# WhatAShot/Electrocardio-Panorama

Measured on AMD Instinct MI355X. Metric: ECG-samples/sec (train step), higher is better.
Workload: dtype f32 (conv products: fp32 operands split into fp16 hi+lo = 22-23 bits, block-scaled, 3 fp16 matrix products each, fp32 accumulate; fp32-class, not IEEE fp32)

## Files before the change

### electrocardio_panorama_amd/_lib.py

```python
import ctypes as C
import os

import torch

_HERE = os.path.dirname(os.path.abspath(__file__))
LIB_PATH = os.path.join(_HERE, "csrc", "libnefnet_hip.so")

NEF_OK = 0
_ERR = {-1: "NEF_E_SHAPE", -2: "NEF_E_NULL", -3: "NEF_E_WORKSPACE", -4: "NEF_E_UNSUPPORTED"}

p = C.c_void_p
i32 = C.c_int
i64 = C.c_int64
f32 = C.c_float
sz = C.c_size_t


class ConvArgs(C.Structure):
    _fields_ = [
        ("x", p), ("wp", p), ("y", p), ("bias", p), ("in_scale", p), ("res", p), ("gate", p), ("mask", p),
        ("x_bs", i64), ("x_gs", i64), ("y_bs", i64), ("y_gs", i64), ("sc_bs", i64), ("sc_gs", i64),
        ("res_bs", i64), ("res_gs", i64), ("gate_bs", i64), ("gate_gs", i64),
        ("B", i32), ("T", i32), ("G", i32), ("Cin_g", i32), ("Cout_g", i32), ("K", i32),
        ("relu", i32), ("gate_scale", f32), ("drop_scale", f32), ("drop_p", f32), ("rng_seed", C.c_uint64),
# ... 46 lines not shown
    "nef_convt2_bwd_weight_ws_bytes": (sz, [i32, i32, i32]),
    "nef_convt2_bwd_weight": (i32, [p, p, p, p, p, sz, i32, i32, i32, i32, i32, p]),
    "nef_theta_mlp_fwd": (i32, [p, p, p, p, i32, i32, p]),
    "nef_theta_mlp_bwd": (i32, [p, p, p, p, i32, i32, p]),
    "nef_theta_encode": (i32, [p, p, i32, p]),
    "nef_chscale_fwd": (i32, [p, p, i64, p, i32, i32, i32, p]),
    "nef_chscale_bwd": (i32, [p, p, p, i64, p, p, i32, i32, i32, i32, p]),
    "nef_gate": (i32, [p, p, p, f32, i64, p]),
    "nef_add": (i32, [p, p, p, i64, p]),
    "nef_roi_align_fwd": (i32, [p, p, p, i32, i32, i32, i32, i32, p]),
    "nef_roi_align_bwd": (i32, [p, p, p, i32, i32, i32, i32, i32, p]),
    "nef_window_crop": (i32, [p, i64, i64, p, i32, i32, i32, i32, i32, i32, p]),
    "nef_window_scatter": (i32, [p, p, i64, i64, i32, i32, i32, i32, i32, i32, p]),
    "nef_roi_unpool_fwd": (i32, [p, p, p, p, i32, i32, i32, p]),
    "nef_roi_unpool_bwd": (i32, [p, p, p, i32, i32, i32, p]),
    "nef_roi_segment_table": (i32, [p, p, p, i32, p]),
    "nef_lead_mean": (i32, [p, p, p, i32, i32, i32, p]),
    "nef_mix_fwd": (i32, [p, p, p, p, p, i32, i32, i32, i32, i32, p, p]),
    "nef_mix_bwd": (i32, [p, p, p, p, p, p, p, p, i32, i32, i32, i32, i32, p, i32, p]),
    "nef_mix_fwd_shared": (i32, [p, p, p, p, p, i32, i32, i32, i32, i32, p, p]),
    "nef_lead_mean_mix_shared": (i32, [p, p, p, p, p, i32, i32, i32, i32, i32, p, p]),
    "nef_mix_bwd_shared_up": (i32, [p, p, p, p, p, p, p, p, i32, i32, i32, i32, i32, p, i32, p]),
    "nef_mix_bwd_shared": (i32, [p, p, p, p, p, p, p, p, i32, i32, i32, i32, i32, p, i32, p]),
    "nef_pass_combine_fwd": (i32, [p, p, p, i32, i32, i32, p]),
    "nef_pass_combine_bwd": (i32, [p, p, i32, i32, i32, p]),
    "nef_pass_combine_stats_ws_bytes": (sz, [i32, i32]),
    "nef_pass_combine_fwd_stats": (i32, [p, p, p, p, p, p, p, p, p, p, p, p, sz, i32, i32, i32, f32, f32, p, p]),
    "nef_mix_bwd_up": (i32, [p, p, p, p, p, p, p, p, i32, i32, i32, i32, i32, p, i32, p]),
    "nef_upsample2_fwd": (i32, [p, p, i64, i32, p]),
    "nef_upsample2_bwd": (i32, [p, p, i64, i32, p]),
    "nef_bn_ws_bytes": (sz, [i32, i32]),
    "nef_bn_train_stats": (i32, [p, p, p, p, p, p, p, p, p, p, sz, i32, i32, i32, i32, f32, f32, p, p]),
    "nef_conv_stats_slots": (i32, [i32, i32]),
    "nef_bn_stats_from_slots": (i32, [p, i32, p, p, p, p, p, p, p, p, p, sz, i32, i32, i32, i32, f32, f32, p, p]),
    "nef_bn_eval_affine": (i32, [p, p, p, p, p, p, i32, f32, p]),
    "nef_fold_bn": (i32, [p, p, p, p, p, p, i32, i32, p]),
    "nef_affine_relu_fwd": (i32, [p, p, p, p, i32, i32, i32, i32, p]),
    "nef_bn_bwd_ws_bytes": (sz, [i32, i32, i32]),
    "nef_bn_relu_bwd": (i32, [p, p, p, p, p, p, p, p, p, p, p, p, sz, i32, i32, i32, i32, p, i32, p]),
    "nef_bn_relu_bwd_phase_major": (i32, [p, p, p, p, p, p, p, p, p, p, p, p, sz, i32, i32, i32, i32, p, i32, p]),
    "nef_bn_relu_bwd_up": (i32, [p, p, p, p, p, p, p, p, p, p, p, sz, i32, i32, i32, i32, p, i32, p]),
    "nef_bn_relu_bwd_combine3": (i32, [p, p, p, p, p, p, p, p, p, p, p, sz, i32, i32, i32, p, i32, p]),
    "nef_bn_relu_bwd_combine3_phase_major": (i32, [p, p, p, p, p, p, p, p, p, p, p, sz, i32, i32, i32, p, i32, p]),
    "nef_bn_bwd_outconv_ws_bytes": (sz, [i32, i32, i32, i32]),
    "nef_bn_relu_bwd_outconv": (i32, [p, p, p, p, p, p, p, p, p, p, p, p, p, sz, i32, i32, i32, i32, p]),
    "nef_outconv_fwd": (i32, [p, p, p, p, i32, i32, i32, p]),
# ... 65 lines not shown
```

### electrocardio_panorama_amd/csrc/roi.hip

```cpp
#include "nef_common.h"

namespace {

constexpr int NSEG = NEF_N_SEG;
constexpr int BINS = NEF_ROI_BINS;
constexpr int SEGW = 2 * NEF_ROI_BINS;

__device__ __forceinline__ int64_t latent_index(int64_t roi) {
    return (int64_t)((float)roi * 0.25f);
}

__device__ __forceinline__ float grid_x(const int64_t* __restrict__ roi_b, int j, int s, int T) {
    const float sc = (float)(2.0 / (double)T);
    const float r0 = ((float)roi_b[2 * j] * 0.25f) * sc + (-1.0f);
    const float r1 = ((float)roi_b[2 * j + 1] * 0.25f) * sc + (-1.0f);
    const float step = (r1 - r0) / (float)(BINS - 1);
    return s < BINS / 2 ? r0 + step * (float)s : r1 - step * (float)(BINS - 1 - s);
}

__device__ __forceinline__ float col_weight(float gx) {
    const float ix = ((gx + 1.f) * 1.f - 1.f) * 0.5f;
    const float x0 = floorf(ix);
    const float we = ix - x0;
    const float ww = 1.f - we;
// ... 71 lines not shown
        if (len < 0) { ok = false; len = 0; }
        if (run + len > T) { ok = false; len = T - run; }
        st.start[j] = (int)a;
        st.len[j] = (int)len;
        st.off[j] = run;
        st.scale[j] = len > 0 ? (float)SEGW / (float)(int)len : 0.f;
        run += (int)len;
    }
    if (run != T) ok = false;
    return ok;
}

__device__ __forceinline__ void lerp_src(int i, float scale, int& i0, int& i1, float& l0, float& l1) {
    float src = scale * ((float)i + 0.5f) - 0.5f;
    if (src < 0.f) src = 0.f;
    i0 = (int)src;
    if (i0 > SEGW - 1) i0 = SEGW - 1;
    i1 = i0 + (i0 < SEGW - 1 ? 1 : 0);
    l1 = src - (float)i0;
    if (l1 < 0.f) l1 = 0.f;
    if (l1 > 1.f) l1 = 1.f;
    l0 = 1.f - l1;
}

__global__ void roi_unpool_fwd_kernel(const float* __restrict__ zseg, const int64_t* __restrict__ rois,
                                      float* __restrict__ out, int32_t* __restrict__ status, int B, int C, int T) {
    const int64_t rows = (int64_t)B * C;
    const int wave = __builtin_amdgcn_readfirstlane((int)(threadIdx.x >> 6)), lane = threadIdx.x & 63;
    const int64_t per_wave = (rows + (int64_t)gridDim.x * 4 - 1) / ((int64_t)gridDim.x * 4);
    const int64_t row_lo = ((int64_t)blockIdx.x * 4 + wave) * per_wave;
    const int64_t row_hi = row_lo + per_wave < rows ? row_lo + per_wave : rows;
    int b_cur = -1;
    SegTable st;
    for (int64_t row = row_lo; row < row_hi; ++row) {
        const int b = (int)(row / C);
        if (b != b_cur) {
            b_cur = b;
            const bool ok = load_segments(rois + (int64_t)b * NSEG * 2, T, st);
            if (!ok && status && lane == 0) status[0] = 1;
        }
        const float* zr = zseg + row * NSEG * SEGW;
        float* orow = out + row * T;
        float r[4];
#pragma unroll
        for (int q = 0; q < 4; ++q) r[q] = (q * 64 + lane < NSEG * SEGW) ? zr[q * 64 + lane] : 0.f;
        int covered = 0;
#pragma unroll
        for (int j = 0; j < NSEG; ++j) {
            const int len = st.len[j], off = st.off[j];
            const float sc = st.scale[j];
            const float reg = r[j >> 1];
            const int base = (j & 1) * SEGW;
            for (int ib = 0; ib < len; ib += 64) {
                const int i = ib + lane;
                int i0, i1;
                float l0, l1;
                lerp_src(i, sc, i0, i1, l0, l1);
                const float v0 = __shfl(reg, base + i0), v1 = __shfl(reg, base + i1);
                if (i < len) orow[off + i] = l0 * v0 + l1 * v1;
            }
            covered = off + len;
        }
        for (int t = covered + lane; t < T; t += 64) orow[t] = 0.f;
    }
}

__device__ __forceinline__ int unpool_left_tap(int i, float scale) {
    float src = scale * ((float)i + 0.5f) - 0.5f;
    if (src < 0.f) src = 0.f;
    return (int)src;
}

__device__ __forceinline__ int unpool_first_reaching(int s, int len, float scale, float inv_scale) {
    if (s <= 0) return 0;
    int i = (int)ceilf(((float)s + 0.5f) * inv_scale - 0.5f);
    if (i < 0) i = 0;
    if (i > len) i = len;
    if (i > 0 && unpool_left_tap(i - 1, scale) >= s) --i;
    else if (i < len && unpool_left_tap(i, scale) < s) ++i;
    if ((i > 0 && unpool_left_tap(i - 1, scale) >= s) || (i < len && unpool_left_tap(i, scale) < s)) {
#pragma nounroll
        while (i > 0 && unpool_left_tap(i - 1, scale) >= s) --i;
// ... 54 lines not shown
                const int b1 = s + 1 < SEGW ? nb : len;
                const int a0 = s > 0 ? pb : b0;
                const float* gp = gr + off;
                float fi = (float)a0 + 0.5f;
                const float sm1 = (float)(s - 1);
                for (int i = a0; i < b0; ++i, fi += 1.f) {
                    float src = sc * fi - 0.5f;
                    src = src < 0.f ? 0.f : src;
                    acc += (src - sm1) * gp[i];
                }
                const float c0 = s == SEGW - 1 ? 1.f : (float)(s + 1), k = s == SEGW - 1 ? 0.f : 1.f;
                for (int i = b0; i < b1; ++i, fi += 1.f) {
                    float src = sc * fi - 0.5f;
                    src = src < 0.f ? 0.f : src;
                    acc += (c0 - k * src) * gp[i];
                }
            }
            gz[j * SEGW + s] = acc;
        }
        if constexpr (STAGED) __builtin_amdgcn_wave_barrier();
    }
}

__global__ void roi_segment_table_kernel(const int64_t* __restrict__ rois, int64_t* __restrict__ seg_start,
                                         int64_t* __restrict__ seg_len, int n) {
    const int i = blockIdx.x * blockDim.x + threadIdx.x;
    if (i >= n) return;
    const int64_t a = latent_index(rois[2 * i]);
    const int64_t e = latent_index(rois[2 * i + 1]);
    seg_start[i] = a;
    seg_len[i] = e - a;
}

}

#define NEF_ST ((hipStream_t)stream)

extern "C" {

static bool window_covers_taps(int T, int zT, int t_off) {
    const int r0 = (T - 1) / 2, r1 = (r0 + 1 < T) ? r0 + 1 : r0;
    return zT > 0 && t_off >= 0 && t_off <= r0 && r1 < t_off + zT && t_off + zT <= T;
}

int nef_roi_align_fwd(const float* z, const int64_t* rois, float* out, int B, int C, int T, int zT, int t_off,
                      nef_stream_t stream) {
// ... 20 lines not shown
                       nef_stream_t stream) {
    NEF_ENTER();
    NEF_REQUIRE(zseg && rois && out, NEF_E_NULL);
    NEF_REQUIRE(B > 0 && C > 0 && T > 0, NEF_E_SHAPE);
    hipLaunchKernelGGL(roi_unpool_fwd_kernel, dim3(nef_stream_grid((int64_t)B * C, 4)), dim3(256), 0, NEF_ST, zseg,
                       rois, out, status, B, C, T);
    return nef_launch_status();
}

int nef_roi_unpool_bwd(const float* gout, const int64_t* rois, float* gzseg, int B, int C, int T,
                       nef_stream_t stream) {
    NEF_ENTER();
    NEF_REQUIRE(gout && rois && gzseg, NEF_E_NULL);
    NEF_REQUIRE(B > 0 && C > 0 && T > 0, NEF_E_SHAPE);
    const dim3 grid(nef_stream_grid((int64_t)B * C, 4));
    if (T <= 4096)
        hipLaunchKernelGGL(roi_unpool_bwd_kernel<true>, grid, dim3(256), (size_t)4 * T * sizeof(float), NEF_ST, gout,
                           rois, gzseg, B, C, T);
    else
        hipLaunchKernelGGL(roi_unpool_bwd_kernel<false>, grid, dim3(256), 0, NEF_ST, gout, rois, gzseg, B, C, T);
    return nef_launch_status();
}

int nef_roi_segment_table(const int64_t* rois, int64_t* seg_start, int64_t* seg_len, int B, nef_stream_t stream) {
    NEF_ENTER();
    NEF_REQUIRE(rois && seg_start && seg_len, NEF_E_NULL);
    NEF_REQUIRE(B > 0, NEF_E_SHAPE);
    const int n = B * NSEG;
    hipLaunchKernelGGL(roi_segment_table_kernel, dim3((n + 255) / 256), dim3(256), 0, NEF_ST, rois, seg_start, seg_len,
                       n);
    return nef_launch_status();
}

}
```

### electrocardio_panorama_amd/engine.py

```python
import os

import torch
from . import _env

from . import ops
from .ops import GV

N_SEG, ROI_BINS = 7, 16
DROP_P = 0.2
BN_EPS, BN_MOM = 1e-5, 0.1


DROPOUT_SITES = ("W_encoder.layer1.0", "W_encoder.layer1.1", "W_encoder.layer1.2", "w_conv.0", "z1_conv.0",
                 "z2_conv1.0", "z2_conv2.0", "z2_conv2.2")


class DropCfg:

    def __init__(self, training, p=DROP_P, masks=None, seed=0, seed_dev=None):
        self.seed_dev = seed_dev
        self.on = bool(training) and p > 0.0
        self.p = p if self.on else 0.0
        self.scale = 1.0 / (1.0 - p) if self.on else 1.0
        self.masks = masks
# ... 357 lines not shown
    else:
        ew = ops.chscale_fwd(a, e)
        enc, sv["blk_w_conv"] = block_fwd(GV.dense(ew, V), P, "w_conv.0", 3, 128, drop)
    z1, sv["blk_z1"] = block_fwd(GV.half(enc, V, 0), P, "z1_conv.0", 3, 128, drop)
    if win is not None:
        xw = ops.window_crop(GV.half(enc, V, 1), win[0], win[1])
        wdrop = drop.windowed("z2_conv1.0", win[0], win[1])
        z2c, sv["blk_z2c"] = block_fwd(GV.dense(xw, V), P, "z2_conv1.0", 3, 128, wdrop)
        z2a = ops.roi_align_fwd(z2c, rois, T, win[0])
    else:
        z2c, sv["blk_z2c"] = block_fwd(GV.half(enc, V, 1), P, "z2_conv1.0", 3, 128, drop)
        z2a = ops.roi_align_fwd(z2c, rois)
    sv["z2_win"] = win
    h0 = z2a.view(B, 128 * V * N_SEG, ROI_BINS)
    h1, sv["blk_c20"] = block_fwd(GV.dense(h0, N_SEG * V), P, "z2_conv2.0", 3, 128, drop)
    h2 = ops.convt2_fwd(h1, P["z2_conv2.1.weight"], P["z2_conv2.1.bias"], N_SEG * V)
    h3, sv["blk_c22"] = block_fwd(GV.dense(h2, N_SEG * V), P, "z2_conv2.2", 3, 128, drop)
    z2b = h3.view(B, 128 * V, N_SEG, 2 * ROI_BINS)
    if save:
        sv.update(x=x, w=a, e=e, in_theta=in_theta, h1=h1, rois=rois, T=T, V=V, B=B)
    return z1, z2b, (sv if save else None)


def _head_fwd(P, Bf, z1, z2r, q_theta, V, rest_theta, phase, training, lead_choice, sv, rest_chunk, half_sweep):
    B = z1.shape[0]
    save = sv is not None
    q = ops.theta_mlp_fwd(q_theta, P["mlp2.weight"], P["mlp2.bias"])
    if 2 * z1.shape[2] >= 128:
        latent, D2 = ops.lead_mean_mix_shared(z1, z2r, q, V, lead_choice)
        out3, dsv = decoder_fwd(D2, P, Bf, 3, training, save, shared_B=B)
    else:
        latent = ops.lead_mean(z1, z2r, V)
        D = ops.mix_fwd(latent, z1, z2r, q, V, lead_choice)
        out3, dsv = decoder_fwd(D, P, Bf, 3, training, save)
    outs = (out3[0:B], out3[B:2 * B], out3[2 * B:3 * B])
    if save:
        sv.update(z1=z1, z2r=z2r, latent=latent, q=q, q_theta=q_theta, choice=lead_choice, dec=dsv, hB=B, hV=V)
    if phase == "train":
        return outs, sv
    if phase in ("val", "test"):
        rest = sweep(P, Bf, latent, rest_theta, training, rest_chunk, half_sweep)
        return outs + (rest,), sv
    raise KeyError("please type correct phase")


def forward(P, Bf, x, in_theta, q_theta, rois, rest_theta=None, phase="train", training=True, drop=None,
            lead_choice=(0, 0), save=False, rest_chunk=8, status=None, half_sweep=False):
    drop = drop or DropCfg(False)
    B, V, L = x.shape
    T = L // 4
    ops.BATCH_HINT = B
    ops.amax_roll()
    pack_side = None
    if save and phase == "train":
        reqs = _step_pack_requests(P, V, T)
        pack_side = _side(x.device, B * 128 * V * T)
        pack_side.run(lambda: ops.pack_many(reqs))
    z1, z2b, sv = _latents(P, x, in_theta, rois, drop, save, pack_side)
    if phase == "gen":
        return (z1, z2b), None
    z2r = ops.roi_unpool_fwd(z2b, rois, T, status)
    return _head_fwd(P, Bf, z1, z2r, q_theta, V, rest_theta, phase, training, lead_choice, sv, rest_chunk, half_sweep)


def _lead_view(t, i, V):
    B, Ct, T = t.shape
    return GV(t, B, 1, 128, T, Ct * T, 128 * T, i * 128 * T)


def forward2(P, Bf, x, in_theta, q_theta, rois, rest_theta=None, phase="train", training=True, drop=None,
             lead_choice=(0, 0), save=False, rest_chunk=8, status=None, half_sweep=False):
    drop = drop or DropCfg(False)
    B, V, L = x.shape
    T, N = L // 4, V * B
    ops.BATCH_HINT = N
    ops.amax_roll()
    xf = x.transpose(0, 1).reshape(N, 1, L).contiguous()
    thf = in_theta.transpose(0, 1).reshape(N, 1, 2).contiguous()
    roisf = rois.repeat(V, 1, 1)
    z1f, z2bf, sv = _latents(P, xf, thf, roisf, drop, save)
    z2rf = ops.roi_unpool_fwd(z2bf, roisf, T, status)
    Z1 = torch.empty(B, 128 * V, T, device=x.device, dtype=torch.float32)
    Z2 = torch.empty_like(Z1)
# ... 87 lines not shown
                             Q * 4 * T, 4 * T)
    return rest


def gen_ecg(P, Bf, z1, z2b, query_thetas, rois, chunk=8, half=False):
    V = z1.shape[1] // 128
    ops.BATCH_HINT = z1.shape[0]
    ops.amax_roll()
    z2r = ops.roi_unpool_fwd(z2b.contiguous(), rois, z1.shape[2])
    latent = ops.lead_mean(z1, z2r, V)
    if half:
        return sweep_eval_h(P, Bf, latent, query_thetas)
    return sweep(P, Bf, latent, query_thetas, False, chunk)


def _head_bwd(P, sv, g_outs, grads, side, relu_z1=False):
    B, V = sv["hB"], sv["hV"]
    like = sv["dec"][2]
    g_out = ops.stacked3(g_outs) if all(g is not None for g in g_outs) else None
    if g_out is None:
        parts = [g if g is not None else torch.zeros_like(like[0:B]) for g in g_outs]
        g_out = torch.cat([p_.contiguous() for p_ in parts], dim=0)
    gD, up, shared = decoder_bwd(sv["dec"], g_out, P, grads, side)
    if shared:
        gz1, gz2r, gq = ops.mix_bwd_shared_up(gD, sv["latent"], sv["z1"], sv["z2r"], sv["q"], V, sv["choice"],
                                              relu_z1=relu_z1)
    else:
        gz1, gz2r, gq = ops.mix_bwd(gD, sv["latent"], sv["z1"], sv["z2r"], sv["q"], V, sv["choice"], upsampled=up,
                                    relu_z1=relu_z1)
    gW2, gb2 = side.run(lambda: ops.theta_mlp_bwd(sv["q_theta"], gq, 256), gq)
    grads["mlp2.weight"], grads["mlp2.bias"] = gW2, gb2
    return gz1, gz2r


EARLY_HOOK = None


def _latents_bwd(P, sv, gz1, gz2r, grads, side, z1_pre_gated=False, early=False):
    B, V, T = sv["B"], sv["V"], sv["T"]
    ops.pack_many(_latent_pack_requests(P, V, T, sv["z2_win"], True))
    gz2b = ops.roi_unpool_bwd(gz2r, sv["rois"])
    gh3 = gz2b.view(B, 128 * V * N_SEG, 2 * ROI_BINS)
    gh2 = block_bwd(sv["blk_c22"], gh3, P, grads, side=side)
    gh2q = ops.convt2_deinterleave(gh2)
    gwt, gbt = side.run(lambda: ops.convt2_bwd_weight(sv["h1"], gh2, N_SEG * V, gyq=gh2q), sv["h1"], gh2, gh2q)
    grads["z2_conv2.1.weight"], grads["z2_conv2.1.bias"] = gwt, gbt
    gh1 = ops.convt2_bwd_data(gh2, P["z2_conv2.1.weight"], N_SEG * V, gyq=gh2q)
    gh0 = block_bwd(sv["blk_c20"], gh1, P, grads, side=side)
    genc = torch.empty(B, 128 * V, T, device=gz1.device, dtype=torch.float32)
    block_bwd(sv["blk_z1"], gz1, P, grads, out=GV.half(genc, V, 0), side=side, pre_gated=z1_pre_gated, gate_input=True)
    win = sv["z2_win"]
    if win is not None:
        gz2c = ops.roi_align_bwd(gh0.view(B, 128 * V, N_SEG, ROI_BINS), sv["rois"], T, win[1], win[0])
        gxw = block_bwd(sv["blk_z2c"], gz2c, P, grads, side=side, gate_input=True)
        ops.window_scatter(gxw, GV.half(genc, V, 1), win[0])
    else:
        gz2c = ops.roi_align_bwd(gh0.view(B, 128 * V, N_SEG, ROI_BINS), sv["rois"], T)
        block_bwd(sv["blk_z2c"], gz2c, P, grads, out=GV.half(genc, V, 1), side=side, gate_input=True)
    gew = block_bwd(sv["blk_w_conv"], genc, P, grads, side=side, pre_gated=True, scale_bwd=True)
    if isinstance(gew, tuple):
        g, ge = gew
    else:
        g, ge = ops.chscale_bwd(gew, sv["w"], sv["e"], relu_x=True)
    gW1, gb1 = side.run(lambda: ops.theta_mlp_bwd(sv["in_theta"], ge, 128), ge)
    grads["mlp1.weight"], grads["mlp1.bias"] = gW1, gb1
    if early:
        if EARLY_HOOK is not None:
            EARLY_HOOK(P, grads, side)
        else:
            from . import parallel
            parallel.early_reduce(P, grads, getattr(side, "stream", None))
    for i in (2, 1, 0):
        g = block_bwd(sv["blk_enc"][i], g, P, grads, side=side, pre_gated=True, gate_input=(i > 0))
    grads["W_encoder.conv1.weight"] = ops.stem_bwd_weight(sv["x"], P["W_encoder.conv1.weight"], g)


def backward(P, sv, g_outs):
    grads = {}
    side = _side(sv["z1"].device, sv["z1"].numel())
    gz1, gz2r = _head_bwd(P, sv, g_outs, grads, side, relu_z1=True)
    _latents_bwd(P, sv, gz1, gz2r, grads, side, z1_pre_gated=True, early=True)
    side.join()
    return grads


def backward2(P, sv, g_outs):
    grads = {}
    side = _side(sv["z1"].device, sv["z1"].numel())
    gZ1, gZ2 = _head_bwd(P, sv, g_outs, grads, side)
    B, V = sv["fold"]
    T = gZ1.shape[2]
    gz1f = torch.empty(V * B, 128, T, device=gZ1.device, dtype=torch.float32)
    gz2rf = torch.empty_like(gz1f)
    for name, gZ, xin, gout in (("single_conv_z1.0", gZ1, sv["z1f"], gz1f), ("single_conv_z2.0", gZ2, sv["z2rf"], gz2rf)):
        wf = ops.pack_weight(P[name + ".weight"], 1, flip=True, T=T)
        gw = None
        for i in range(V):
            gv = _lead_view(gZ, i, V)
            ops.conv(gv, wf, 128, 3, out=GV.dense(gout[i * B:(i + 1) * B], 1), role="conv_bwd_data")
            w = ops.conv_bwd_weight(GV.dense(xin[i * B:(i + 1) * B], 1), gv, 3)
            gw = w if gw is None else ops.add(gw, w)
        cs = ops.chan_sum(gZ)
        gb = cs[0:128].contiguous()
        for i in range(1, V):
            gb = ops.add(gb, cs[i * 128:(i + 1) * 128].contiguous())
        grads[name + ".weight"], grads[name + ".bias"] = gw, gb
    _latents_bwd(P, sv, gz1f, gz2rf, grads, side)
    side.join()
    return grads
```

### electrocardio_panorama_amd/ops.py

```python
import ctypes as C
import contextlib
import itertools
import os

import torch
from . import _env

from . import _lib

N_SEG, ROI_BINS = 7, 16


def _p(t):
    return None if t is None else t.data_ptr()


def _stream():
    return torch.cuda.current_stream().cuda_stream


def _chk(t, dtype=torch.float32):
    assert t.is_cuda and t.dtype == dtype and t.is_contiguous(), (t.device, t.dtype, t.is_contiguous())
    return t

# ... 1105 lines not shown
               "nef_lead_mean_mix_shared")
    _done(ev)
    return latent, D2


def mix_bwd_shared_up(gU2, latent, z1, z2r, q, V, c1, c2=None, relu_z1=False):
    L = _lib.load()
    c1, c2, cdev = _choice(c1 if c2 is None else (c1, c2))
    _chk(gU2)
    B, _, T = latent.shape
    up = gU2.shape[2] == 2 * T
    assert gU2.shape == (2 * B, 256, 2 * T if up else T)
    gz1, gz2r = torch.empty_like(z1), torch.empty_like(z2r)
    gq = torch.empty(B, 256, device=latent.device, dtype=torch.float32)
    name = "mix_bwd_shared_up" if up else "mix_bwd_shared"
    ev = _hbm(name, gU2, z1, z2r, gz1, gz2r)
    fn = L.nef_mix_bwd_shared_up if up else L.nef_mix_bwd_shared
    _lib.check(fn(_p(gU2), _p(latent), _p(z1), _p(z2r), _p(q), _p(gz1), _p(gz2r), _p(gq), B, V, T, c1, c2, cdev, int(relu_z1),
                  _stream()), "nef_" + name)
    _done(ev)
    return gz1, gz2r, gq


def pass_combine_fwd(P2, bias, B):
    L = _lib.load()
    _chk(P2), _chk(bias)
    C2, Ln = P2.shape[1], P2.shape[2]
    c1 = torch.empty(3 * B, C2 // 2, Ln, device=P2.device, dtype=torch.float32)
    ev = _hbm("pass_combine_fwd", P2, c1)
    _lib.check(L.nef_pass_combine_fwd(_p(P2), _p(bias), _p(c1), B, C2 // 2, Ln, _stream()), "nef_pass_combine_fwd")
    _done(ev)
    return c1


def pass_combine_fwd_stats(P2, bias, B, gamma, beta, running_mean, running_var, eps=1e-5, momentum=0.1, nbt=None):
    L = _lib.load()
    _chk(P2), _chk(bias)
    C2, Ln = P2.shape[1], P2.shape[2]
    Ct = C2 // 2
    c1 = torch.empty(3 * B, Ct, Ln, device=P2.device, dtype=torch.float32)
    mean, invstd, a, b = (torch.empty(3, Ct, device=P2.device, dtype=torch.float32) for _ in range(4))
    n = L.nef_pass_combine_stats_ws_bytes(B, Ct)
    ws = workspace(n, P2.device)
    ev = _hbm("pass_combine_fwd", P2, c1)
    _lib.check(L.nef_pass_combine_fwd_stats(_p(P2), _p(bias), _p(c1), _p(gamma), _p(beta), _p(running_mean),
                                            _p(running_var), _p(mean), _p(invstd), _p(a), _p(b), _p(ws), n, B, Ct, Ln, eps,
# ... 395 lines not shown
```

### include/nefnet_hip.h

```cpp
#ifndef NEFNET_HIP_H
#define NEFNET_HIP_H

#include <stddef.h>
#include <stdint.h>

#ifdef __cplusplus
extern "C" {
#endif

#define NEF_OK 0
#define NEF_E_SHAPE (-1)
#define NEF_E_NULL (-2)
#define NEF_E_WORKSPACE (-3)
#define NEF_E_UNSUPPORTED (-4)

#define NEF_N_SEG 7
#define NEF_ROI_BINS 16

typedef void* nef_stream_t;

int nef_abi_version(void);

int nef_debug_spin_us(float us, int wgs, nef_stream_t stream);

// ... 143 lines not shown
                       nef_stream_t stream);
int nef_roi_segment_table(const int64_t* rois, int64_t* seg_start, int64_t* seg_len, int B, nef_stream_t stream);

int nef_lead_mean(const float* z1, const float* z2r, float* latent, int B, int V, int T, nef_stream_t stream);
int nef_mix_fwd(const float* latent, const float* z1, const float* z2r, const float* q, float* D, int B, int V,
                int T, int c1, int c2, const int32_t* choice_dev, nef_stream_t stream);
int nef_mix_bwd(const float* gD, const float* latent, const float* z1, const float* z2r, const float* q, float* gz1,
                float* gz2r, float* gq, int B, int V, int T, int c1, int c2, const int32_t* choice_dev, int relu_z1,
                nef_stream_t stream);
int nef_mix_bwd_up(const float* gU, const float* latent, const float* z1, const float* z2r, const float* q, float* gz1,
                float* gz2r, float* gq, int B, int V, int T, int c1, int c2, const int32_t* choice_dev, int relu_z1,
                nef_stream_t stream);

int nef_mix_fwd_shared(const float* latent, const float* z1, const float* z2r, const float* q, float* D2, int B, int V,
                       int T, int c1, int c2, const int32_t* choice_dev, nef_stream_t stream);
int nef_lead_mean_mix_shared(const float* z1, const float* z2r, const float* q, float* latent, float* D2, int B, int V,
                             int T, int c1, int c2, const int32_t* choice_dev, nef_stream_t stream);
int nef_mix_bwd_shared(const float* gD2, const float* latent, const float* z1, const float* z2r, const float* q,
                       float* gz1, float* gz2r, float* gq, int B, int V, int T, int c1, int c2,
                       const int32_t* choice_dev, int relu_z1, nef_stream_t stream);
int nef_mix_bwd_shared_up(const float* gU2, const float* latent, const float* z1, const float* z2r, const float* q,
                          float* gz1, float* gz2r, float* gq, int B, int V, int T, int c1, int c2,
                          const int32_t* choice_dev, int relu_z1, nef_stream_t stream);
int nef_pass_combine_fwd(const float* P2, const float* bias, float* c1, int B, int C, int L, nef_stream_t stream);
size_t nef_pass_combine_stats_ws_bytes(int B, int C);
int nef_pass_combine_fwd_stats(const float* P2, const float* bias, float* c1, const float* gamma, const float* beta,
                               float* running_mean, float* running_var, float* mean, float* invstd, float* a, float* b,
                               void* ws, size_t ws_bytes, int B, int C, int L, float eps, float momentum,
                               int64_t* num_batches_tracked, nef_stream_t stream);
int nef_pass_combine_bwd(const float* gc1, float* gP2, int B, int C, int L, nef_stream_t stream);

int nef_upsample2_fwd(const float* x, float* y, int64_t N, int Tin, nef_stream_t stream);
int nef_upsample2_bwd(const float* gy, float* gx, int64_t N, int Tin, nef_stream_t stream);

size_t nef_bn_ws_bytes(int P, int C);
int nef_conv_stats_slots(int T, int Cout_g);
int nef_bn_stats_from_slots(const float* slots, int nslot, const float* gamma, const float* beta, float* running_mean,
                            float* running_var, float* mean, float* invstd, float* a, float* b, void* ws,
                            size_t ws_bytes, int P, int Bp, int C, int L, float eps, float momentum,
                            int64_t* num_batches_tracked, nef_stream_t stream);
int nef_bn_train_stats(const float* x, const float* gamma, const float* beta, float* running_mean,
                       float* running_var, float* mean, float* invstd, float* a, float* b, void* ws, size_t ws_bytes,
                       int P, int Bp, int C, int L, float eps, float momentum, int64_t* num_batches_tracked,
                       nef_stream_t stream);
int nef_bn_eval_affine(const float* gamma, const float* beta, const float* running_mean, const float* running_var,
                       float* a, float* b, int C, float eps, nef_stream_t stream);
// ... 95 lines not shown
```

Measured before the change: 8690.

## Fuse ROI unpooling into lead-mean mix forward and mix backward kernels

Adds fused kernels that compute the ROI unpool of z2b on the fly inside the lead-mean/mix forward and the mix backward, staging segment rows in LDS per wave. This avoids materializing the unpooled z2r tensor and running a separate roi_unpool backward, cutting HBM traffic and kernel launches. The backward writes gz2b directly by gathering through segment tables. The cost is more per-element interpolation work, LDS usage that limits occupancy, and a fallback path that recomputes the unpool when the decoder is upsampled.

```diff
diff --git a/electrocardio_panorama_amd/_lib.py b/electrocardio_panorama_amd/_lib.py
--- a/electrocardio_panorama_amd/_lib.py
+++ b/electrocardio_panorama_amd/_lib.py
@@ -92,6 +92,8 @@
     "nef_lead_mean_mix_shared": (i32, [p, p, p, p, p, i32, i32, i32, i32, i32, p, p]),
     "nef_mix_bwd_shared_up": (i32, [p, p, p, p, p, p, p, p, i32, i32, i32, i32, i32, p, i32, p]),
     "nef_mix_bwd_shared": (i32, [p, p, p, p, p, p, p, p, i32, i32, i32, i32, i32, p, i32, p]),
+    "nef_lead_mean_mix_unpool": (i32, [p, p, p, p, p, p, p, i32, i32, i32, i32, i32, p, p]),
+    "nef_mix_bwd_unpool": (i32, [p, p, p, p, p, p, p, p, p, i32, i32, i32, i32, i32, p, i32, p]),
     "nef_pass_combine_fwd": (i32, [p, p, p, i32, i32, i32, p]),
     "nef_pass_combine_bwd": (i32, [p, p, i32, i32, i32, p]),
     "nef_pass_combine_stats_ws_bytes": (sz, [i32, i32]),
diff --git a/electrocardio_panorama_amd/csrc/roi.hip b/electrocardio_panorama_amd/csrc/roi.hip
--- a/electrocardio_panorama_amd/csrc/roi.hip
+++ b/electrocardio_panorama_amd/csrc/roi.hip
@@ -117,6 +117,8 @@
     if (l1 > 1.f) l1 = 1.f;
     l0 = 1.f - l1;
 }
+
+__device__ __forceinline__ float unpool_tap(float l0, float v0, float l1, float v1) { return l0 * v0 + l1 * v1; }
 
 __global__ void roi_unpool_fwd_kernel(const float* __restrict__ zseg, const int64_t* __restrict__ rois,
                                       float* __restrict__ out, int32_t* __restrict__ status, int B, int C, int T) {
@@ -152,7 +154,7 @@
                 float l0, l1;
                 lerp_src(i, sc, i0, i1, l0, l1);
                 const float v0 = __shfl(reg, base + i0), v1 = __shfl(reg, base + i1);
-                if (i < len) orow[off + i] = l0 * v0 + l1 * v1;
+                if (i < len) orow[off + i] = unpool_tap(l0, v0, l1, v1);
             }
             covered = off + len;
         }
@@ -253,6 +255,359 @@
     }
 }
 
+constexpr int SEGROW = NSEG * SEGW;
+
+typedef float roi_f32x2 __attribute__((ext_vector_type(2)));
+
+__device__ __forceinline__ void stage_segment_rows(const float* __restrict__ zb, float* __restrict__ zs, int V, int lane) {
+    for (int v = 0; v < V; ++v)
+#pragma unroll
+        for (int q = 0; q < 4; ++q)
+            if (q * 64 + lane < SEGROW) zs[v * SEGROW + q * 64 + lane] = zb[(int64_t)v * 128 * SEGROW + q * 64 + lane];
+    __builtin_amdgcn_fence(__ATOMIC_RELEASE, "wavefront");
+    __builtin_amdgcn_wave_barrier();
+}
+
+template <int FORM>
+__global__ __launch_bounds__(256) void lead_mean_mix_unpool_kernel(const float* __restrict__ z1, const float* __restrict__ z2b,
+                                                                   const int64_t* __restrict__ rois, const float* __restrict__ q,
+                                                                   float* __restrict__ latent, float* __restrict__ D2,
+                                                                   int32_t* __restrict__ status, int B, int V, int T, int c1, int c2,
+                                                                   const int32_t* __restrict__ choice_dev) {
+    extern __shared__ float head_lds[];
+    if (choice_dev) { c1 = choice_dev[0]; c2 = choice_dev[1]; }
+    const int nw = (int)(blockDim.x >> 6);
+    const int wave = __builtin_amdgcn_readfirstlane((int)(threadIdx.x >> 6)), lane = threadIdx.x & 63;
+    const float fv = (float)V;
+    const int64_t n1 = (int64_t)B * (FORM == 2 ? 64 : 128), n2 = (int64_t)B * 128;
+    const int64_t rowsT = (int64_t)B * 256 * T;
+    float* zs = head_lds + wave * V * SEGROW;
+    int b_cur = -1;
+    SegTable st;
+    for (int64_t it = (int64_t)blockIdx.x * nw + wave; it < n1 + n2; it += (int64_t)gridDim.x * nw) {
+        if (it < n1) {
+            if constexpr (FORM == 2) {
+                typedef float vec __attribute__((ext_vector_type(4)));
+                const int b = (int)(it >> 6), c = 2 * (int)(it & 63);
+                const int64_t row = (int64_t)b * 256 + c;
+                const int TW = T / 2, mid = T / 4;
+                const int64_t lead = (int64_t)128 * T / 4, pass = (int64_t)B * 128 * TW;
+                const vec* src = (const vec*)(z1 + ((int64_t)b * V * 128 + c) * T);
+                const float f0 = q[row], f1 = q[row + 1];
+                vec* lat = latent ? (vec*)latent + (row >> 1) * TW : nullptr;
+                vec* d0 = (vec*)D2 + (row >> 1) * TW;
+                int t = lane;
+                for (; t + 64 < TW; t += 128) {
+                    vec s0 = src[t], s1 = src[t + 64];
+                    vec p0 = s0, p1 = s1;
+                    for (int v = 1; v < V; ++v) {
+                        const vec x0 = src[(int64_t)v * lead + t], x1 = src[(int64_t)v * lead + t + 64];
+                        s0 += x0;
+                        s1 += x1;
+                        if (v == c1) { p0 = x0; p1 = x1; }
+                    }
+                    const vec m0 = s0 / fv, m1 = s1 / fv;
+                    const vec g0 = t < mid ? vec{f0, f0, f0, f0} : (t > mid ? vec{f1, f1, f1, f1} : vec{f0, f0, f1, f1});
+                    const vec g1 = t + 64 < mid ? vec{f0, f0, f0, f0} : (t + 64 > mid ? vec{f1, f1, f1, f1} : vec{f0, f0, f1, f1});
+                    if (lat) { lat[t] = m0; lat[t + 64] = m1; }
+                    d0[t] = g0 * m0;
+                    d0[t + 64] = g1 * m1;
+                    d0[pass + t] = g0 * p0;
+                    d0[pass + t + 64] = g1 * p1;
+                }
+                for (; t < TW; t += 64) {
+                    vec sm = src[t];
+                    vec pk = sm;
+                    for (int v = 1; v < V; ++v) {
+                        const vec x = src[(int64_t)v * lead + t];
+                        sm += x;
+                        if (v == c1) pk = x;
+                    }
+                    const vec m = sm / fv;
+                    const vec g0 = t < mid ? vec{f0, f0, f0, f0} : (t > mid ? vec{f1, f1, f1, f1} : vec{f0, f0, f1, f1});
+                    if (lat) lat[t] = m;
+                    d0[t] = g0 * m;
+                    d0[pass + t] = g0 * pk;
+                }
+            } else {
+                constexpr int W = FORM + 1;
+                typedef float vec __attribute__((ext_vector_type(W)));
+                const int b = (int)(it >> 7), c = (int)(it & 127);
+                const int64_t row = (int64_t)b * 256 + c;
+                const int TW = T / W;
+                const int64_t lead = (int64_t)128 * TW, pass = (int64_t)B * 256 * TW;
+                const vec* src = (const vec*)(z1 + ((int64_t)b * V * 128 + c) * T);
+                const float f = q[row];
+                vec* lat = latent ? (vec*)latent + row * TW : nullptr;
+                vec* d0 = (vec*)D2 + row * TW;
+                for (int t = lane; t < TW; t += 64) {
+                    vec s = src[t];
+                    vec pk = s;
+                    for (int v = 1; v < V; ++v) {
+                        const vec x = src[(int64_t)v * lead + t];
+                        s += x;
+                        if (v == c1) pk = x;
+                    }
+                    const vec m = s / fv;
+                    if (lat) lat[t] = m;
+                    d0[t] = f * m;
+                    d0[pass + t] = f * pk;
+                }
+            }
+            continue;
+        }
+        const int64_t k = it - n1;
+        const int b = (int)(k >> 7), cc = (int)(k & 127);
+        if (b != b_cur) {
+            b_cur = b;
+            const bool ok = load_segments(rois + (int64_t)b * NSEG * 2, T, st);
+            if (!ok && status && lane == 0) status[0] = 1;
+        }
+        __builtin_amdgcn_wave_barrier();
+        stage_segment_rows(z2b + ((int64_t)b * V * 128 + cc) * SEGROW, zs, V, lane);
+        const int64_t row = (int64_t)b * 256 + 128 + cc;
+        const float f = q[row];
+        float* lat = latent ? latent + row * T : nullptr;
+        float* d0 = D2 + row * T;
+        float* d1 = d0 + rowsT;
+        int covered = 0;
+#pragma unroll
+        for (int j = 0; j < NSEG; ++j) {
+            const int len = st.len[j], off = st.off[j];
+            const float sc = st.scale[j];
+            const float* sp = zs + j * SEGW;
+            for (int i = lane; i < len; i += 64) {
+                int i0, i1;
+                float l0, l1;
+                lerp_src(i, sc, i0, i1, l0, l1);
+                float s = unpool_tap(l0, sp[i0], l1, sp[i1]);
+                float pk = s;
+                for (int v = 1; v < V; ++v) {
+                    const float x = unpool_tap(l0, sp[v * SEGROW + i0], l1, sp[v * SEGROW + i1]);
+                    s += x;
+                    if (v == c2) pk = x;
+                }
+                const float m = s / fv;
+                if (lat) lat[off + i] = m;
+                d0[off + i] = f * m;
+                d1[off + i] = f * pk;
+            }
+            covered = off + len;
+        }
+        for (int t = covered + lane; t < T; t += 64) {
+            if (lat) lat[t] = 0.f;
+            d0[t] = d1[t] = f * 0.f;
+        }
+    }
+}
+
+template <bool PAIR>
+__global__ __launch_bounds__(256) void mix_bwd_unpool_kernel(const float* __restrict__ gD, const float* __restrict__ latent,
+                                                             const float* __restrict__ z1, const float* __restrict__ z2b,
+                                                             const int64_t* __restrict__ rois, const float* __restrict__ q,
+                                                             float* __restrict__ gz1, float* __restrict__ gz2b,
+                                                             float* __restrict__ gq, int B, int V, int T, int c1, int c2,
+                                                             const int32_t* __restrict__ choice_dev, int relu_z1) {
+    extern __shared__ float head_lds[];
+    if (choice_dev) { c1 = choice_dev[0]; c2 = choice_dev[1]; }
+    const int nw = (int)(blockDim.x >> 6);
+    const int wave = __builtin_amdgcn_readfirstlane((int)(threadIdx.x >> 6)), lane = threadIdx.x & 63;
+    const float fv = (float)V;
+    const int64_t n1 = (int64_t)B * (PAIR ? 64 : 128), n2 = (int64_t)B * 128;
+    const int64_t rowsT = (int64_t)B * 256 * T;
+    float* zs = head_lds + (int64_t)wave * (V * SEGROW + 2 * T);
+    float* stripA = zs + V * SEGROW;
+    float* stripB = stripA + T;
+    const bool mask = relu_z1 != 0, need_z = mask || !latent;
+    int b_cur = -1;
+    SegTable st;
+    for (int64_t it = (int64_t)blockIdx.x * nw + wave; it < n1 + n2; it += (int64_t)gridDim.x * nw) {
+        if (it < n1) {
+            if constexpr (PAIR) {
+                typedef float vec __attribute__((ext_vector_type(4)));
+                const int b = (int)(it >> 6), c = 2 * (int)(it & 63);
+                const int64_t row = (int64_t)b * 256 + c;
+                const int TW = T / 2, mid = T / 4;
+                const int64_t lead = (int64_t)128 * T / 4, gpass = (int64_t)B * 128 * TW;
+                const float f0 = q[row], f1 = q[row + 1];
+                const vec* lat = latent ? (const vec*)latent + (row >> 1) * TW : nullptr;
+                const vec* zsrc = (const vec*)(z1 + ((int64_t)b * V * 128 + c) * T);
+                vec* gdst = (vec*)(gz1 + ((int64_t)b * V * 128 + c) * T);
+                const vec* g0 = (const vec*)gD + (row >> 1) * TW;
+                const vec* g1r = g0 + gpass;
+                float acc0 = 0.f, acc1 = 0.f;
+                for (int t = lane; t < TW; t += 64) {
+                    const vec ga = g0[t], gb = g1r[t];
+                    const vec fq = t < mid ? vec{f0, f0, f0, f0} : (t > mid ? vec{f1, f1, f1, f1} : vec{f0, f0, f1, f1});
+                    vec sm = vec{0.f, 0.f, 0.f, 0.f}, pk = sm;
+                    for (int v = 0; v < V; ++v) {
+                        vec o;
+#pragma unroll
+                        for (int e = 0; e < 4; ++e) o[e] = fq[e] * ga[e] / fv + (v == c1 ? fq[e] * gb[e] : 0.f);
+                        if (need_z || v == c1) {
+                            const vec z = zsrc[(int64_t)v * lead + t];
+                            if (v == 0) sm = z; else sm += z;
+                            if (v == c1) pk = z;
+                            if (mask) {
+#pragma unroll
+                                for (int e = 0; e < 4; ++e)
+                                    if (!(z[e] > 0.f)) o[e] = 0.f;
+                            }
+                        }
+                        gdst[(int64_t)v * lead + t] = o;
+                    }
+                    const vec l4 = lat ? lat[t] : sm / fv;
+#pragma unroll
+                    for (int e = 0; e < 4; ++e) {
+                        const float term = ga[e] * l4[e] + gb[e] * pk[e];
+                        if (t < mid || (t == mid && e < 2)) acc0 += term; else acc1 += term;
+                    }
+                }
+                acc0 = nef_wave_sum(acc0);
+                acc1 = nef_wave_sum(acc1);
+                if (lane == 0) { gq[row] = acc0; gq[row + 1] = acc1; }
+            } else {
+                const int b = (int)(it >> 7), c = (int)(it & 127);
+                const int64_t row = (int64_t)b * 256 + c;
+                const float f = q[row];
+                const float* lat = latent ? latent + row * T : nullptr;
+                const float* zsrc = z1 + ((int64_t)b * V * 128 + c) * T;
+                float* gdst = gz1 + ((int64_t)b * V * 128 + c) * T;
+                const float* g0 = gD + row * T;
+                const int G = ((T & 1) == 0 && T >= 8) ? 2 : 1;
+                float acc = 0.f;
+                for (int p = lane; p * G < T; p += 64) {
+                    for (int e = 0; e < G; ++e) {
+                        const int t = p * G + e;
+                        const float ga = g0[t], gb = g0[rowsT + t];
+                        const float gm = f * ga / fv;
+                        float sm = 0.f, pk = 0.f;
+                        for (int v = 0; v < V; ++v) {
+                            float o = gm + (v == c1 ? f * gb : 0.f);
+                            if (need_z || v == c1) {
+                                const float z = zsrc[(int64_t)v * 128 * T + t];
+                                if (v == 0) sm = z; else sm += z;
+                                if (v == c1) pk = z;
+                                if (mask && !(z > 0.f)) o = 0.f;
+                            }
+                            gdst[(int64_t)v * 128 * T + t] = o;
+                        }
+                        const float l = lat ? lat[t] : sm / fv;
+                        acc += ga * l + gb * pk;
+                    }
+                }
+                acc = nef_wave_sum(acc);
+                if (lane == 0) gq[row] = acc;
+            }
+            continue;
+        }
+        const int64_t k = it - n1;
+        const int b = (int)(k >> 7), cc = (int)(k & 127);
+        if (b != b_cur) {
+            b_cur = b;
+            load_segments(rois + (int64_t)b * NSEG * 2, T, st);
+        }
+        __builtin_amdgcn_wave_barrier();
+        stage_segment_rows(z2b + ((int64_t)b * V * 128 + cc) * SEGROW, zs, V, lane);
+        const int64_t row = (int64_t)b * 256 + 128 + cc;
+        const float f = q[row];
+        const float* lat = latent ? latent + row * T : nullptr;
+        const float* g0 = gD + row * T;
+        const float* g1r = g0 + rowsT;
+        const int G = PAIR ? 4 : (((T & 1) == 0 && T >= 8) ? 2 : 1);
+        const int r0 = PAIR ? (cc & 1) * T : 0;
+        const int t_lo = r0 / G, t_hi = (r0 + T + G - 1) / G;
+        float acc = 0.f;
+        for (int t = (t_lo & ~63) + lane; t < t_hi; t += 64) {
+            if (t < t_lo) continue;
+            const int ib = G * t - r0;
+            float gav[4] = {0.f, 0.f, 0.f, 0.f}, gbv[4] = {0.f, 0.f, 0.f, 0.f};
+            if (G == 1) {
+                gav[0] = g0[ib];
+                gbv[0] = g1r[ib];
+            } else {
+#pragma unroll
+                for (int h = 0; h < 2; ++h) {
+                    const int ih = ib + 2 * h;
+                    if (2 * h < G && ih >= 0 && ih < T) {
+                        const roi_f32x2 a2 = *(const roi_f32x2*)(g0 + ih), b2 = *(const roi_f32x2*)(g1r + ih);
+                        gav[2 * h] = a2[0]; gav[2 * h + 1] = a2[1];
+                        gbv[2 * h] = b2[0]; gbv[2 * h + 1] = b2[1];
+                    }
+                }
+            }
+#pragma unroll
+            for (int e = 0; e < 4; ++e) {
+                const int i = ib + e;
+                if (e >= G || i < 0 || i >= T) continue;
+                int len = 0, off = 0, base = 0;
+                float sc = 0.f;
+#pragma unroll
+                for (int j = 0; j < NSEG; ++j)
+                    if (i >= st.off[j] && i < st.off[j] + st.len[j]) { len = st.len[j]; off = st.off[j]; sc = st.scale[j]; base = j * SEGW; }
+                if (len == 0) continue;
+                const float ga = gav[e], gb = gbv[e];
+                const float* sp = zs + base;
+                int i0, i1;
+                float l0, l1;
+                lerp_src(i - off, sc, i0, i1, l0, l1);
+                const float pk = unpool_tap(l0, sp[c2 * SEGROW + i0], l1, sp[c2 * SEGROW + i1]);
+                float l;
+                if (lat) {
+                    l = lat[i];
+                } else {
+                    float sm = unpool_tap(l0, sp[i0], l1, sp[i1]);
+                    for (int v = 1; v < V; ++v) sm += unpool_tap(l0, sp[v * SEGROW + i0], l1, sp[v * SEGROW + i1]);
+                    l = sm / fv;
+                }
+                acc += ga * l + gb * pk;
+                const float gm = f * ga / fv;
+                stripA[i] = gm;
+                stripB[i] = gm + f * gb;
+            }
+        }
+        acc = nef_wave_sum(acc);
+        if (lane == 0) gq[row] = acc;
+        __builtin_amdgcn_fence(__ATOMIC_RELEASE, "wavefront");
+        __builtin_amdgcn_wave_barrier();
+        const int s = lane & (SEGW - 1), half = lane >> 5;
+        float* gz = gz2b + ((int64_t)b * V * 128 + cc) * SEGROW;
+#pragma unroll
+        for (int jj = 0; jj < NSEG + 1; jj += 2) {
+            const int j = jj + half;
+            if (j >= NSEG) continue;
+            const int len = half ? st.len[jj + 1 < NSEG ? jj + 1 : jj] : st.len[jj];
+            const int off = half ? st.off[jj + 1 < NSEG ? jj + 1 : jj] : st.off[jj];
+            const float sc = half ? st.scale[jj + 1 < NSEG ? jj + 1 : jj] : st.scale[jj];
+            float accA = 0.f, accB = 0.f;
+            if (len > 0) {
+                const int b0 = unpool_first_reaching(s, len, sc, (float)len * (1.f / SEGW));
+                const int nb = __shfl_down(b0, 1), pb = __shfl_up(b0, 1);
+                const int b1 = s + 1 < SEGW ? nb : len;
+                const int a0 = s > 0 ? pb : b0;
+                const float* gpA = stripA + off;
+                const float* gpB = stripB + off;
+                float fi = (float)a0 + 0.5f;
+                const float sm1 = (float)(s - 1);
+                for (int i = a0; i < b0; ++i, fi += 1.f) {
+                    float src = sc * fi - 0.5f;
+                    src = src < 0.f ? 0.f : src;
+                    accA += (src - sm1) * gpA[i];
+                    accB += (src - sm1) * gpB[i];
+                }
+                const float c0 = s == SEGW - 1 ? 1.f : (float)(s + 1), kk = s == SEGW - 1 ? 0.f : 1.f;
+                for (int i = b0; i < b1; ++i, fi += 1.f) {
+                    float src = sc * fi - 0.5f;
+                    src = src < 0.f ? 0.f : src;
+                    accA += (c0 - kk * src) * gpA[i];
+                    accB += (c0 - kk * src) * gpB[i];
+                }
+            }
+            for (int v = 0; v < V; ++v) gz[(int64_t)v * 128 * SEGROW + j * SEGW + s] = v == c2 ? accB : accA;
+        }
+    }
+}
+
 __global__ void roi_segment_table_kernel(const int64_t* __restrict__ rois, int64_t* __restrict__ seg_start,
                                          int64_t* __restrict__ seg_len, int n) {
     const int i = blockIdx.x * blockDim.x + threadIdx.x;
@@ -319,6 +674,59 @@
     return nef_launch_status();
 }
 
+static int head_waves(size_t wave_bytes) {
+    for (int nw = 4; nw >= 1; nw >>= 1)
+        if (nw * wave_bytes <= 65536) return nw;
+    return 0;
+}
+
+int nef_lead_mean_mix_unpool(const float* z1, const float* z2b, const int64_t* rois, const float* q, float* latent,
+                             float* D2, int32_t* status, int B, int V, int T, int c1, int c2, const int32_t* choice_dev,
+                             nef_stream_t stream) {
+    NEF_ENTER();
+    NEF_REQUIRE(z1 && z2b && rois && q && D2, NEF_E_NULL);
+    NEF_REQUIRE(B > 0 && V > 0 && T > 0 && c1 >= 0 && c1 < V && c2 >= 0 && c2 < V, NEF_E_SHAPE);
+    const size_t wave_bytes = (size_t)V * SEGROW * sizeof(float);
+    const int nw = head_waves(wave_bytes);
+    NEF_REQUIRE(nw > 0, NEF_E_SHAPE);
+    const bool al16 = (((uintptr_t)z1 | (uintptr_t)latent | (uintptr_t)D2) & 15) == 0;
+    const int form = (T % 4 == 2 && al16) ? 2 : (T % 2 == 0 ? 1 : 0);
+    const dim3 grid(nef_stream_grid((int64_t)B * (form == 2 ? 192 : 256), nw)), block(64 * nw);
+    const size_t lds = nw * wave_bytes;
+    if (form == 2)
+        hipLaunchKernelGGL(lead_mean_mix_unpool_kernel<2>, grid, block, lds, NEF_ST, z1, z2b, rois, q, latent, D2, status, B, V, T,
+                           c1, c2, choice_dev);
+    else if (form == 1)
+        hipLaunchKernelGGL(lead_mean_mix_unpool_kernel<1>, grid, block, lds, NEF_ST, z1, z2b, rois, q, latent, D2, status, B, V, T,
+                           c1, c2, choice_dev);
+    else
+        hipLaunchKernelGGL(lead_mean_mix_unpool_kernel<0>, grid, block, lds, NEF_ST, z1, z2b, rois, q, latent, D2, status, B, V, T,
+                           c1, c2, choice_dev);
+    return nef_launch_status();
+}
+
+int nef_mix_bwd_unpool(const float* gD2, const float* latent, const float* z1, const float* z2b, const int64_t* rois,
+                       const float* q, float* gz1, float* gz2b, float* gq, int B, int V, int T, int c1, int c2,
+                       const int32_t* choice_dev, int relu_z1, nef_stream_t stream) {
+    NEF_ENTER();
+    NEF_REQUIRE(gD2 && z1 && z2b && rois && q && gz1 && gz2b && gq, NEF_E_NULL);
+    NEF_REQUIRE(B > 0 && V > 0 && T > 1 && T <= 4096 && c1 >= 0 && c1 < V && c2 >= 0 && c2 < V, NEF_E_SHAPE);
+    const size_t wave_bytes = ((size_t)V * SEGROW + 2 * (size_t)T) * sizeof(float);
+    const int nw = head_waves(wave_bytes);
+    NEF_REQUIRE(nw > 0, NEF_E_SHAPE);
+    const bool al16 = (((uintptr_t)gD2 | (uintptr_t)latent | (uintptr_t)z1 | (uintptr_t)gz1) & 15) == 0;
+    const bool pair = T % 4 == 2 && T >= 8 && al16;
+    const dim3 grid(nef_stream_grid((int64_t)B * (pair ? 192 : 256), nw)), block(64 * nw);
+    const size_t lds = nw * wave_bytes;
+    if (pair)
+        hipLaunchKernelGGL(mix_bwd_unpool_kernel<true>, grid, block, lds, NEF_ST, gD2, latent, z1, z2b, rois, q, gz1, gz2b, gq, B, V,
+                           T, c1, c2, choice_dev, relu_z1);
+    else
+        hipLaunchKernelGGL(mix_bwd_unpool_kernel<false>, grid, block, lds, NEF_ST, gD2, latent, z1, z2b, rois, q, gz1, gz2b, gq, B, V,
+                           T, c1, c2, choice_dev, relu_z1);
+    return nef_launch_status();
+}
+
 int nef_roi_segment_table(const int64_t* rois, int64_t* seg_start, int64_t* seg_len, int B, nef_stream_t stream) {
     NEF_ENTER();
     NEF_REQUIRE(rois && seg_start && seg_len, NEF_E_NULL);
diff --git a/electrocardio_panorama_amd/engine.py b/electrocardio_panorama_amd/engine.py
--- a/electrocardio_panorama_amd/engine.py
+++ b/electrocardio_panorama_amd/engine.py
@@ -403,11 +403,15 @@
     return z1, z2b, (sv if save else None)
 
 
-def _head_fwd(P, Bf, z1, z2r, q_theta, V, rest_theta, phase, training, lead_choice, sv, rest_chunk, half_sweep):
+def _head_fwd(P, Bf, z1, z2r, q_theta, V, rest_theta, phase, training, lead_choice, sv, rest_chunk, half_sweep, unpool=None):
     B = z1.shape[0]
     save = sv is not None
     q = ops.theta_mlp_fwd(q_theta, P["mlp2.weight"], P["mlp2.bias"])
-    if 2 * z1.shape[2] >= 128:
+    if unpool is not None:
+        latent, D2 = ops.lead_mean_mix_unpool(z1, unpool[0], unpool[1], q, V, lead_choice, status=unpool[2],
+                                              want_latent=phase != "train")
+        out3, dsv = decoder_fwd(D2, P, Bf, 3, training, save, shared_B=B)
+    elif 2 * z1.shape[2] >= 128:
         latent, D2 = ops.lead_mean_mix_shared(z1, z2r, q, V, lead_choice)
         out3, dsv = decoder_fwd(D2, P, Bf, 3, training, save, shared_B=B)
     else:
@@ -416,7 +420,8 @@
         out3, dsv = decoder_fwd(D, P, Bf, 3, training, save)
     outs = (out3[0:B], out3[B:2 * B], out3[2 * B:3 * B])
     if save:
-        sv.update(z1=z1, z2r=z2r, latent=latent, q=q, q_theta=q_theta, choice=lead_choice, dec=dsv, hB=B, hV=V)
+        sv.update(z1=z1, z2r=z2r, latent=latent, q=q, q_theta=q_theta, choice=lead_choice, dec=dsv, hB=B, hV=V,
+                  unpool=None if unpool is None else unpool[:2])
     if phase == "train":
         return outs, sv
     if phase in ("val", "test"):
@@ -440,6 +445,9 @@
     z1, z2b, sv = _latents(P, x, in_theta, rois, drop, save, pack_side)
     if phase == "gen":
         return (z1, z2b), None
+    if 2 * T >= 128 and ops.head_unpool_covers(V, T):
+        return _head_fwd(P, Bf, z1, None, q_theta, V, rest_theta, phase, training, lead_choice, sv, rest_chunk, half_sweep,
+                         unpool=(z2b, rois, status))
     z2r = ops.roi_unpool_fwd(z2b, rois, T, status)
     return _head_fwd(P, Bf, z1, z2r, q_theta, V, rest_theta, phase, training, lead_choice, sv, rest_chunk, half_sweep)
 
@@ -573,24 +581,32 @@
         parts = [g if g is not None else torch.zeros_like(like[0:B]) for g in g_outs]
         g_out = torch.cat([p_.contiguous() for p_ in parts], dim=0)
     gD, up, shared = decoder_bwd(sv["dec"], g_out, P, grads, side)
-    if shared:
-        gz1, gz2r, gq = ops.mix_bwd_shared_up(gD, sv["latent"], sv["z1"], sv["z2r"], sv["q"], V, sv["choice"],
-                                              relu_z1=relu_z1)
-    else:
-        gz1, gz2r, gq = ops.mix_bwd(gD, sv["latent"], sv["z1"], sv["z2r"], sv["q"], V, sv["choice"], upsampled=up,
-                                    relu_z1=relu_z1)
+    gz2b = None
+    latent, z2r = sv["latent"], sv["z2r"]
+    if sv.get("unpool") is not None and up:
+        z2r = ops.roi_unpool_fwd(sv["unpool"][0], sv["unpool"][1], sv["z1"].shape[2])
+        latent = latent if latent is not None else ops.lead_mean(sv["z1"], z2r, V)
+    if z2r is None:
+        gz1, gz2b, gq = ops.mix_bwd_unpool(gD, latent, sv["z1"], sv["unpool"][0], sv["unpool"][1], sv["q"], V, sv["choice"],
+                                           relu_z1=relu_z1)
+        gz2r = None
+    elif shared:
+        gz1, gz2r, gq = ops.mix_bwd_shared_up(gD, latent, sv["z1"], z2r, sv["q"], V, sv["choice"], relu_z1=relu_z1)
+    else:
+        gz1, gz2r, gq = ops.mix_bwd(gD, latent, sv["z1"], z2r, sv["q"], V, sv["choice"], upsampled=up, relu_z1=relu_z1)
     gW2, gb2 = side.run(lambda: ops.theta_mlp_bwd(sv["q_theta"], gq, 256), gq)
     grads["mlp2.weight"], grads["mlp2.bias"] = gW2, gb2
-    return gz1, gz2r
+    return gz1, gz2r, gz2b
 
 
 EARLY_HOOK = None
 
 
-def _latents_bwd(P, sv, gz1, gz2r, grads, side, z1_pre_gated=False, early=False):
+def _latents_bwd(P, sv, gz1, gz2r, grads, side, z1_pre_gated=False, early=False, gz2b=None):
     B, V, T = sv["B"], sv["V"], sv["T"]
     ops.pack_many(_latent_pack_requests(P, V, T, sv["z2_win"], True))
-    gz2b = ops.roi_unpool_bwd(gz2r, sv["rois"])
+    if gz2b is None:
+        gz2b = ops.roi_unpool_bwd(gz2r, sv["rois"])
     gh3 = gz2b.view(B, 128 * V * N_SEG, 2 * ROI_BINS)
     gh2 = block_bwd(sv["blk_c22"], gh3, P, grads, side=side)
     gh2q = ops.convt2_deinterleave(gh2)
@@ -629,8 +645,8 @@
 def backward(P, sv, g_outs):
     grads = {}
     side = _side(sv["z1"].device, sv["z1"].numel())
-    gz1, gz2r = _head_bwd(P, sv, g_outs, grads, side, relu_z1=True)
-    _latents_bwd(P, sv, gz1, gz2r, grads, side, z1_pre_gated=True, early=True)
+    gz1, gz2r, gz2b = _head_bwd(P, sv, g_outs, grads, side, relu_z1=True)
+    _latents_bwd(P, sv, gz1, gz2r, grads, side, z1_pre_gated=True, early=True, gz2b=gz2b)
     side.join()
     return grads
 
@@ -638,7 +654,7 @@
 def backward2(P, sv, g_outs):
     grads = {}
     side = _side(sv["z1"].device, sv["z1"].numel())
-    gZ1, gZ2 = _head_bwd(P, sv, g_outs, grads, side)
+    gZ1, gZ2, _ = _head_bwd(P, sv, g_outs, grads, side)
     B, V = sv["fold"]
     T = gZ1.shape[2]
     gz1f = torch.empty(V * B, 128, T, device=gZ1.device, dtype=torch.float32)
diff --git a/electrocardio_panorama_amd/ops.py b/electrocardio_panorama_amd/ops.py
--- a/electrocardio_panorama_amd/ops.py
+++ b/electrocardio_panorama_amd/ops.py
@@ -1151,6 +1151,40 @@
     return gz1, gz2r, gq
 
 
+def head_unpool_covers(V, T):
+    return 1 < T <= 4096 and (224 * V + 2 * T) * 4 <= 65536
+
+
+def lead_mean_mix_unpool(z1, z2b, rois, q, V, c1, c2=None, status=None, want_latent=True):
+    L = _lib.load()
+    c1, c2, cdev = _choice(c1 if c2 is None else (c1, c2))
+    _chk(z1), _chk(z2b), _chk(q), _chk(rois, torch.int64)
+    B, _, T = z1.shape
+    assert z2b.shape == (B, 128 * V, N_SEG, 2 * ROI_BINS)
+    latent = torch.empty(B, 256, T, device=z1.device, dtype=torch.float32) if want_latent else None
+    D2 = torch.empty(2 * B, 256, T, device=z1.device, dtype=torch.float32)
+    ev = _hbm("lead_mean_mix_unpool", z1, z2b, latent, D2)
+    _lib.check(L.nef_lead_mean_mix_unpool(_p(z1), _p(z2b), _p(rois), _p(q), _p(latent), _p(D2), _p(status), B, V, T, c1, c2, cdev,
+                                          _stream()), "nef_lead_mean_mix_unpool")
+    _done(ev)
+    return latent, D2
+
+
+def mix_bwd_unpool(gD2, latent, z1, z2b, rois, q, V, c1, c2=None, relu_z1=False):
+    L = _lib.load()
+    c1, c2, cdev = _choice(c1 if c2 is None else (c1, c2))
+    _chk(gD2), _chk(z1), _chk(z2b), _chk(q), _chk(rois, torch.int64)
+    B, _, T = z1.shape
+    assert gD2.shape == (2 * B, 256, T) and z2b.shape == (B, 128 * V, N_SEG, 2 * ROI_BINS)
+    gz1, gz2b = torch.empty_like(z1), torch.empty_like(z2b)
+    gq = torch.empty(B, 256, device=z1.device, dtype=torch.float32)
+    ev = _hbm("mix_bwd_unpool", gD2, latent, z1, z2b, gz1, gz2b)
+    _lib.check(L.nef_mix_bwd_unpool(_p(gD2), _p(latent), _p(z1), _p(z2b), _p(rois), _p(q), _p(gz1), _p(gz2b), _p(gq), B, V, T, c1, c2,
+                                    cdev, int(relu_z1), _stream()), "nef_mix_bwd_unpool")
+    _done(ev)
+    return gz1, gz2b, gq
+
+
 def pass_combine_fwd(P2, bias, B):
     L = _lib.load()
     _chk(P2), _chk(bias)
diff --git a/include/nefnet_hip.h b/include/nefnet_hip.h
--- a/include/nefnet_hip.h
+++ b/include/nefnet_hip.h
@@ -189,6 +189,12 @@
 int nef_mix_bwd_shared_up(const float* gU2, const float* latent, const float* z1, const float* z2r, const float* q,
                           float* gz1, float* gz2r, float* gq, int B, int V, int T, int c1, int c2,
                           const int32_t* choice_dev, int relu_z1, nef_stream_t stream);
+int nef_lead_mean_mix_unpool(const float* z1, const float* z2b, const int64_t* rois, const float* q, float* latent,
+                             float* D2, int32_t* status, int B, int V, int T, int c1, int c2, const int32_t* choice_dev,
+                             nef_stream_t stream);
+int nef_mix_bwd_unpool(const float* gD2, const float* latent, const float* z1, const float* z2b, const int64_t* rois,
+                       const float* q, float* gz1, float* gz2b, float* gq, int B, int V, int T, int c1, int c2,
+                       const int32_t* choice_dev, int relu_z1, nef_stream_t stream);
 int nef_pass_combine_fwd(const float* P2, const float* bias, float* c1, int B, int C, int L, nef_stream_t stream);
 size_t nef_pass_combine_stats_ws_bytes(int B, int C);
 int nef_pass_combine_fwd_stats(const float* P2, const float* bias, float* c1, const float* gamma, const float* beta,
```

Measured after the change: 8839, median of 6. +1.7%, better.
